# RIKEN-RCCS/EigenExa

Hardware: AMD Instinct MI355X
Metric: eigen_sx full-solve throughput (reference flop model: 4/3 N^3 + D&C GEMM + 2 nvec N^2) (higher is better)
Workload: dtype f64; 1 GPU; N=8192 random symmetric fp64 (counter-based R+R^T, seed 20240807), eigen_sx all eigenpairs, m_forward=64, m_backward=128; parallelism=1 GPU (1x1 grid)

## Files before the change

### eigenexa_amd/csrc/api.hip

```cpp
#include "eigx_context.h"
#include "eigx_comm.h"
#include "../../include/eigenexa_amd.h"
#include <cstring>

namespace eigx {
Context g_ctx;
}

using namespace eigx;

extern "C" {

int eigx_init(int device) {
  return eigx_init_multi(device, 0, 1, nullptr, 'C');
}

int eigx_get_device_count(void) {
  int ndev = 0;
  if (hipGetDeviceCount(&ndev) != hipSuccess) { (void)hipGetLastError(); return 0; }
  return ndev;
}

int eigx_get_rccl_unique_id(void* out128) {
  return comm_get_unique_id(out128);
// ... 269 lines not shown
  for (size_t q = 0; q < g_ctx.prof_kind.size(); ++q) {
    const int k = g_ctx.prof_kind[q];
    if (k < 0 || k >= nkinds) continue;
    float ms = 0.f;
    EIGX_HIP_CHECK(hipEventElapsedTime(&ms, g_ctx.prof_ev[2 * q], g_ctx.prof_ev[2 * q + 1]));
    out[3 * k + 0] += 1.0;
    out[3 * k + 1] += g_ctx.prof_units[q];
    out[3 * k + 2] += 1e-3 * ms;
  }
  return EIGX_OK;
}

int eigx_device_synchronize(void) {
  if (!g_ctx.initialized) return EIGX_ERR_NOT_INITIALIZED;
  EIGX_HIP_CHECK(hipSetDevice(g_ctx.device));
  EIGX_HIP_CHECK(hipDeviceSynchronize());
  return EIGX_OK;
}

void* eigx_malloc_dev(int64_t bytes) {
  if (!g_ctx.initialized) return nullptr;
  void* p = nullptr;
  if (hipMalloc(&p, (size_t)bytes) != hipSuccess) return nullptr;
  return p;
}
int eigx_free_dev(void* p) {
  if (p) EIGX_HIP_CHECK(hipFree(p));
  return EIGX_OK;
}
int eigx_memcpy_h2d(void* dst, const void* src, int64_t bytes) {
  EIGX_HIP_CHECK(hipMemcpy(dst, src, (size_t)bytes, hipMemcpyHostToDevice));
  return EIGX_OK;
}
int eigx_memcpy_d2h(void* dst, const void* src, int64_t bytes) {
  EIGX_HIP_CHECK(hipMemcpy(dst, src, (size_t)bytes, hipMemcpyDeviceToHost));
  return EIGX_OK;
}

int eigx_tune(int key, int value) {
  if (key == 0) return set_gemm_variant(value);
  if (key == 1) return set_bisect_threads(value);
  if (key == 2) return set_bt_q(value);
  if (key == 3 || key == 4 || key == 5 || key == 10 || key == 11) return set_reduce_knob(key, value);
  if (key == 6) return set_gemm_cstream(value);
  if (key == 7) return value > 0 ? set_reduce_knob(key, value) : -1;
  if (key == 8) return set_dc_chunk(value);
  if (key == 9) return comm_set_bounce(value);
  if (key == 15) return set_dc_pipe(value);
  if (key == 16) return set_dc_batch(value);
  if (key == 17 || key == 18 || key == 19) return set_range_knob(key, value);
  if (key == 20) return set_tri_nb(value);
  if (key == 21) return set_batch_nmax(value);
  if (key == 22) return set_hbatch_nmax(value);
  return -1;
}

int eigx_dgemm_dev(char opa, char opb, int m, int n, int k, double alpha, const double* a, int lda,
                   const double* b, int ldb, double beta, double* c, int ldc, int tri_upper) {
  if (!g_ctx.initialized) return EIGX_ERR_NOT_INITIALIZED;
  EIGX_HIP_CHECK(hipStreamSynchronize(nullptr));
  dgemm_dev(g_ctx.stream, opa, opb, m, n, k, alpha, a, lda, b, ldb, beta, c, ldc, tri_upper ? 1 : 0,
            &g_ctx.grid);
  EIGX_HIP_CHECK(hipStreamSynchronize(g_ctx.stream));
  return EIGX_OK;
}

int eigx_dgemm_gather_dev(char opa, char opb, int m, int n, int k, double alpha, const double* a, int lda,
                          const double* b, int ldb, double beta, double* c, int ldc, const int* kmap_a,
                          const int* kmap_b) {
  if (!g_ctx.initialized) return EIGX_ERR_NOT_INITIALIZED;
  EIGX_HIP_CHECK(hipStreamSynchronize(nullptr));
  dgemm_dev(g_ctx.stream, opa, opb, m, n, k, alpha, a, lda, b, ldb, beta, c, ldc, 0, nullptr, kmap_a, nullptr, 1, 0,
            0, 0, 1, 0, 0, 0, 1, 0, kmap_b);
  EIGX_HIP_CHECK(hipStreamSynchronize(g_ctx.stream));
  return EIGX_OK;
}

}
```

### eigenexa_amd/csrc/dc.hip

```cpp
#include "eigx_context.h"
#include "eigx_comm.h"
#include "../../include/eigenexa_amd.h"
#include <algorithm>
#include <cfloat>
#include <cstring>

namespace eigx {

namespace {

constexpr int LEAF = 32;

constexpr int LEAF_T = 64;
__global__ __launch_bounds__(LEAF_T) void jacobi_leaf_kernel(const double* __restrict__ d,
                                                             const double* __restrict__ e, int lde, int band,
                                                             const int* __restrict__ leaf_off,
                                                             const int* __restrict__ leaf_n, double* __restrict__ D,
                                                             double* __restrict__ Q, int ldq, int r0, int r1) {
  __shared__ double A[LEAF][LEAF + 1];
  __shared__ double V[LEAF][LEAF + 1];
  __shared__ double cs[LEAF / 2][2];
  __shared__ int pq[LEAF / 2][2];
  __shared__ int perm[LEAF];
  const int tid = threadIdx.x;
// ... 202 lines not shown
  const int jj = blockIdx.x * blockDim.x + threadIdx.x;
  if (jj >= M.nm) return;
  double v = 0.0;
  if (jj < M.K) {
    const int nch = (M.K + ZN_IC - 1) / ZN_IC;
    for (int c = 0; c < nch; ++c) v += zp[(size_t)c * ldn + M.off + jj];
  } else {
    const double* col = Qa + (size_t)dsrc[M.off + jj] * ldq;
    for (int t = 0; t < M.zr_n; ++t) v += M.zr_w[t] * col[M.zr_row[t]];
  }
  z[M.off + jj] = v;
}

__global__ void pack_rows_kernel(const double* __restrict__ Q, int ldq, int n, int r0, int nr, int rp,
                                 double* __restrict__ out) {
  const int j = blockIdx.y;
  for (int r = blockIdx.x * blockDim.x + threadIdx.x; r < rp; r += gridDim.x * blockDim.x)
    out[(size_t)j * rp + r] = (r < nr) ? Q[(size_t)j * ldq + r0 + r] : 0.0;
}
__global__ void unpack_rows_kernel(const double* __restrict__ in, int n, int rp, double* __restrict__ Q, int ldq) {
  const int j = blockIdx.y, q = blockIdx.z;
  const double* src = in + (size_t)q * rp * n + (size_t)j * rp;
  for (int r = blockIdx.x * blockDim.x + threadIdx.x; r < rp; r += gridDim.x * blockDim.x)
    if (q * rp + r < n) Q[(size_t)j * ldq + q * rp + r] = src[r];
}

template <int CTRL>
__device__ __forceinline__ double dc_dpp_add(double v) {
  const int lo2 = __builtin_amdgcn_update_dpp(0, __double2loint(v), CTRL, 0xf, 0xf, true);
  const int hi2 = __builtin_amdgcn_update_dpp(0, __double2hiint(v), CTRL, 0xf, 0xf, true);
  return v + __hiloint2double(hi2, lo2);
}

__device__ __forceinline__ double dc_swapadd16(double v) {
  const auto lo = __builtin_amdgcn_permlane16_swap(__double2loint(v), __double2loint(v), false, false);
  const auto hi = __builtin_amdgcn_permlane16_swap(__double2hiint(v), __double2hiint(v), false, false);
  return __hiloint2double(hi[0], lo[0]) + __hiloint2double(hi[1], lo[1]);
}

__device__ __forceinline__ double group8_sum(double v) {
  v = dc_dpp_add<0xB1>(v);
  v = dc_dpp_add<0x4E>(v);
  v = dc_dpp_add<0x141>(v);
  return v;
}

template <int LPR>
__device__ __forceinline__ double group_sum(double v) {
  v = group8_sum(v);
  if (LPR == 32) { v = dc_dpp_add<0x140>(v); v = dc_swapadd16(v); }
  return v;
}

template <int LPR>
__global__ __launch_bounds__(256) void secular_kernel(const MergeDev* __restrict__ md,
                                                      const double* __restrict__ dlam,
                                                      const double* __restrict__ wz, double* __restrict__ Dn,
                                                      double* __restrict__ S, int lds, int P, int rank,
                                                      double* __restrict__ sec, int nsec) {
  const MergeDev M = md[blockIdx.y];
  const int K = M.K;
  constexpr int RPW = 256 / LPR;
  __shared__ double so[RPW], stau[RPW];
  const int jbase = (P > 1) ? (int)((long)K * rank / P) : 0;
  const int jend = (P > 1) ? (int)((long)K * (rank + 1) / P) : K;
  if (jbase + (int)(blockIdx.x * RPW) >= jend) return;
  const int sub = threadIdx.x & (LPR - 1);
  const int jraw = jbase + blockIdx.x * RPW + threadIdx.x / LPR;
  const bool act = jraw < jend;
  const int j = act ? jraw : K - 1;
  const double* __restrict__ d = dlam + M.off;
  const double* __restrict__ z = wz + M.off;
  double* Sp = S + (size_t)M.off * lds + M.off;
  const double rho = M.rho, rhoinv = 1.0 / rho;
  const double eps = DBL_EPSILON / 2.0;
  if (K == 1) {
    if (threadIdx.x == 0) {
      const double t = rho * z[0] * z[0];
      if (sec) { sec[M.off] = d[0] + t; sec[nsec + M.off] = d[0]; sec[2 * nsec + M.off] = t; }
      else { Dn[M.off] = d[0] + t; Sp[0] = -t; }
    }
    return;
  }
  const bool last = (j == K - 1);
  const int jl = last ? K - 2 : j, jr = jl + 1;
  double origin, lo, hi, tau;
  {
    const double gap = last ? rho : d[j + 1] - d[j];
    const double base = last ? d[K - 1] : d[j], half = 0.5 * gap;
    double c = 0.0;
    for (int i = sub; i < K; i += LPR)
      if (i != jl && i != jr) c += z[i] * z[i] / ((d[i] - base) - half);
    c = group_sum<LPR>(c) + rhoinv;
    const double zl2 = z[jl] * z[jl], zr2 = z[jr] * z[jr];
    const double fmid = c + zl2 / ((d[jl] - base) - half) + zr2 / ((d[jr] - base) - half);
    int org;
    if (last) { org = K - 1; if (fmid <= 0.0) { lo = 0.5 * gap; hi = gap; } else { lo = 0.0; hi = 0.5 * gap; } }
    else if (fmid > 0.0) { org = j; lo = 0.0; hi = 0.5 * gap; }
    else { org = j + 1; lo = -0.5 * gap; hi = 0.0; }
    origin = d[org];
    const double dl = d[jl] - origin, dr = d[jr] - origin;
    const double qa = c, qb = -(c * (dl + dr) + zl2 + zr2), qc = c * dl * dr + zl2 * dr + zr2 * dl;
    tau = 0.5 * (lo + hi);
    const double disc = qb * qb - 4.0 * qa * qc;
    if (disc >= 0.0) {
      const double sq = sqrt(disc);
      const double qq = -0.5 * (qb + (qb >= 0.0 ? sq : -sq));
      const double r1 = (qa != 0.0) ? qq / qa : NAN, r2 = (qq != 0.0) ? qc / qq : NAN;
      if (r1 > lo && r1 < hi) tau = r1;
      else if (r2 > lo && r2 < hi) tau = r2;
    }
  }
  for (int iter = 0; iter < 100; ++iter) {
    double psi = 0.0, dpsi = 0.0, phi = 0.0, dphi = 0.0, err = 0.0;
    for (int i = sub; i < K; i += LPR) {
      const double t = z[i] / ((d[i] - origin) - tau);
      const double zt = z[i] * t, tt = t * t;
      if (i <= jl) { psi += zt; dpsi += tt; err += fabs(psi); }
      else { phi += zt; dphi += tt; err += fabs(phi); }
    }
    psi = group_sum<LPR>(psi); dpsi = group_sum<LPR>(dpsi);
    phi = group_sum<LPR>(phi); dphi = group_sum<LPR>(dphi);
    err = group_sum<LPR>(err);
    const double wv = rhoinv + phi + psi;
    err = 8.0 * (fabs(phi) + fabs(psi)) + err + 2.0 * rhoinv + fabs(tau) * (dpsi + dphi);
    if (fabs(wv) <= eps * err) break;
    if (wv < 0.0) lo = tau; else hi = tau;
    const double Dl = (d[jl] - origin) - tau, Dr = (d[jr] - origin) - tau;
    const double aa = (Dl + Dr) * wv - Dl * Dr * (dpsi + dphi);
    const double bb = Dl * Dr * wv;
    const double cc = wv - Dl * dpsi - Dr * dphi;
    double eta;
    {
      double disc = aa * aa - 4.0 * bb * cc;
      if (disc < 0.0) disc = 0.0;
      const double sq = sqrt(disc);
      if (cc == 0.0) eta = (aa != 0.0) ? bb / aa : 0.0;
      else if (aa <= 0.0) eta = (aa - sq) / (2.0 * cc);
      else eta = 2.0 * bb / (aa + sq);
    }
    if (wv * eta >= 0.0) eta = -wv / (dpsi + dphi);
    double tnew = tau + eta;
    if (!(tnew > lo && tnew < hi)) tnew = 0.5 * (lo + hi);
    if (tnew == tau) break;
    tau = tnew;
  }
  if (sec) {
    if (sub == 0 && act) { sec[M.off + j] = origin + tau; sec[nsec + M.off + j] = origin; sec[2 * nsec + M.off + j] = tau; }
    return;
  }
  if (sub == 0) { so[threadIdx.x / LPR] = origin; stau[threadIdx.x / LPR] = tau; if (act) Dn[M.off + j] = origin + tau; }
  __syncthreads();
  {
    const int r = threadIdx.x % RPW, ii = threadIdx.x / RPW;
    const int jr = blockIdx.x * RPW + r;
    if (jr < K) {
      const double o_ = so[r], t_ = stau[r];
      for (int i = ii; i < K; i += 256 / RPW) Sp[jr + (size_t)i * lds] = (d[i] - o_) - t_;
    }
  }
}

__global__ __launch_bounds__(256) void loewner_kernel(const MergeDev* __restrict__ md,
                                                      const double* __restrict__ dlam,
                                                      const double* __restrict__ wz, const double* __restrict__ S,
                                                      int lds, double* __restrict__ zh) {
  const MergeDev M = md[blockIdx.y];
  const int K = M.K;
  const int lane = threadIdx.x & 63;
  const int i = blockIdx.x * 4 + (threadIdx.x >> 6);
  if (i >= K) return;
  const double* d = dlam + M.off;
  const double* Sp = S + (size_t)M.off * lds + M.off + (size_t)i * lds;
  const double di = d[i];
  double prod = 1.0;
  for (int j = lane; j < K; j += 64) {
    const double num = -Sp[j];
    prod *= (j == i) ? num : num / (d[j] - di);
  }
  for (int o = 32; o > 0; o >>= 1) prod *= __shfl_xor(prod, o, 64);
  if (lane == 0) {
    const double v = sqrt(fabs(prod));
    zh[M.off + i] = (wz[M.off + i] >= 0.0) ? v : -v;
  }
}

constexpr int VEC_IC = 256;
__global__ __launch_bounds__(256) void vectors1_kernel(const MergeDev* __restrict__ md, const double* __restrict__ zh,
                                                       double* __restrict__ S, int lds, double* __restrict__ vnp,
                                                       int ldn) {
  __shared__ double part[4][64];
  const MergeDev M = md[blockIdx.z];
  const int K = M.K;
  if ((int)(blockIdx.x * 64) >= K || (int)(blockIdx.y * VEC_IC) >= K) return;
  const int lane = threadIdx.x & 63, wave = threadIdx.x >> 6;
  const int j = blockIdx.x * 64 + lane;
  const bool act = j < K;
  double* Sp = S + (size_t)M.off * lds + M.off + j;
  const double* zz = zh + M.off;
  const int i0 = blockIdx.y * VEC_IC;
  const int i1 = (i0 + VEC_IC < K) ? i0 + VEC_IC : K;
  double nrm = 0.0;
  if (act)
    for (int i = i0 + wave; i < i1; i += 4) {
      const double v = zz[i] / Sp[(size_t)i * lds];
      Sp[(size_t)i * lds] = v;
      nrm += v * v;
    }
  part[wave][lane] = nrm;
  __syncthreads();
  if (wave == 0 && act)
    vnp[(size_t)blockIdx.y * ldn + M.off + j] = (part[0][lane] + part[1][lane]) + (part[2][lane] + part[3][lane]);
}
__global__ __launch_bounds__(256) void vectors2_kernel(const MergeDev* __restrict__ md, double* __restrict__ S, int lds,
                                                       const double* __restrict__ vnp, int ldn) {
  const MergeDev M = md[blockIdx.z];
  const int K = M.K;
  if ((int)(blockIdx.x * 64) >= K || (int)(blockIdx.y * VEC_IC) >= K) return;
  const int lane = threadIdx.x & 63, wave = threadIdx.x >> 6;
  const int j = blockIdx.x * 64 + lane;
  if (j >= K) return;
  const int nch = (K + VEC_IC - 1) / VEC_IC;
  double nrm = 0.0;
  for (int c = 0; c < nch; ++c) nrm += vnp[(size_t)c * ldn + M.off + j];
  const double sc = 1.0 / sqrt(nrm);
  double* Sp = S + (size_t)M.off * lds + M.off + j;
  const int i0 = blockIdx.y * VEC_IC;
  const int i1 = (i0 + VEC_IC < K) ? i0 + VEC_IC : K;
  for (int i = i0 + wave; i < i1; i += 4) Sp[(size_t)i * lds] *= sc;
}

__global__ void scatter_lambda_kernel(const MergeDev* __restrict__ md, const double* __restrict__ sec, double* __restrict__ Dn) {
  const MergeDev M = md[blockIdx.y];
  const int j = blockIdx.x * blockDim.x + threadIdx.x;
  if (j < M.K) Dn[M.off + j] = sec[M.off + j];
}
__global__ __launch_bounds__(256) void loewner_mg_kernel(const MergeDev* __restrict__ md, const double* __restrict__ dlam,
                                                         const double* __restrict__ wz, const double* __restrict__ sec,
                                                         int nsec, double* __restrict__ zh) {
  const MergeDev M = md[blockIdx.y];
  const int K = M.K;
  const int lane = threadIdx.x & 63;
  const int i = blockIdx.x * 4 + (threadIdx.x >> 6);
  if (i >= K) return;
  const double* d = dlam + M.off;
  const double* org = sec + nsec + M.off;
  const double* tau = sec + 2 * nsec + M.off;
  const double di = d[i];
  double prod = 1.0;
  for (int j = lane; j < K; j += 64) {
    const double num = (org[j] - di) + tau[j];
    prod *= (j == i) ? num : num / (d[j] - di);
  }
  for (int o = 32; o > 0; o >>= 1) prod *= __shfl_xor(prod, o, 64);
  if (lane == 0) {
    const double v = sqrt(fabs(prod));
    zh[M.off + i] = (wz[M.off + i] >= 0.0) ? v : -v;
  }
}
__global__ __launch_bounds__(256) void vectors_mg_kernel(const MergeDev* __restrict__ md, int mi0, const double* __restrict__ dlam,
                                                         const double* __restrict__ zh, const double* __restrict__ sec, int nsec,
                                                         int j0, int j1, int compact, double* __restrict__ Sc, int ldsc) {
  __shared__ double part[4][64];
  const MergeDev M = md[mi0 + blockIdx.z];
  const int K = M.K;
  const int jhi = (j1 < K) ? j1 : K;
  const int lane = threadIdx.x & 63, wave = threadIdx.x >> 6;
  const int j = j0 + blockIdx.x * 64 + lane;
  if (j0 + (int)(blockIdx.x * 64) >= jhi) return;
  const bool act = j < jhi;
  const double* d = dlam + M.off;
  const double* zz = zh + M.off;
  const double oj = act ? sec[nsec + M.off + j] : 0.0, tj = act ? sec[2 * nsec + M.off + j] : 1.0;
  double nrm = 0.0;
  for (int i = wave; i < K; i += 4) {
    const double v = zz[i] / ((d[i] - oj) - tj);
    nrm += v * v;
  }
  part[wave][lane] = nrm;
  __syncthreads();
  const double sc = 1.0 / sqrt((part[0][lane] + part[1][lane]) + (part[2][lane] + part[3][lane]));
  if (!act) return;
// ... 99 lines not shown
        }
      nodes[id].sig[k] = sig[k];
      for (int r = 0; r < band; ++r) {
        nodes[id].wv[k][r] = y[band * k + r];
        nodes[id].wv[k][band + r] = x[band * k + r];
      }
    }
    const int l = build(off, n1);
    const int r = build(off + n1, nn - n1);
    nodes[id].left = l; nodes[id].right = r;
    nodes[l].parent = id; nodes[r].parent = id;
    nodes[id].height = 1 + std::max(nodes[l].height, nodes[r].height);
    return id;
  }
};

void sort_index_runs(const double* d, int nm, std::vector<int>& idx, std::vector<int>& tmp, std::vector<int>& bounds) {
  idx.resize(nm);
  for (int i = 0; i < nm; ++i) idx[i] = i;
  bounds.clear();
  bounds.push_back(0);
  for (int i = 1; i < nm; ++i)
    if (d[i] < d[i - 1]) bounds.push_back(i);
  bounds.push_back(nm);
  auto cmp = [d](int a, int b) { return d[a] < d[b] || (d[a] == d[b] && a < b); };
  int nr = (int)bounds.size() - 1;
  if (nr > 16) { std::sort(idx.begin(), idx.end(), cmp); return; }
  tmp.resize(nm);
  while (nr > 1) {
    int w = 0;
    for (int r = 0; r < nr; r += 2) {
      if (r + 1 < nr)
        std::merge(idx.begin() + bounds[r], idx.begin() + bounds[r + 1], idx.begin() + bounds[r + 1], idx.begin() + bounds[r + 2],
                   tmp.begin() + bounds[r], cmp);
      else
        std::copy(idx.begin() + bounds[r], idx.begin() + bounds[r + 1], tmp.begin() + bounds[r]);
      bounds[w++] = bounds[r];
    }
    bounds[w] = nm;
    nr = w;
    idx.swap(tmp);
  }
}

}

int g_dc_pipe = 1, g_dc_batch = 1, g_dc_side_min = 1024;
int set_dc_pipe(int v) {
  const int old = g_dc_pipe;
  if (v >= 2) g_dc_side_min = v; else g_dc_pipe = v ? 1 : 0;
  return old;
}
int set_dc_batch(int v) { const int old = g_dc_batch; g_dc_batch = v ? 1 : 0; return old; }
int g_dc_chunk = 2048;
int set_dc_chunk(int v) {
  const int old = g_dc_chunk;
  if (v >= 64 && v <= 2048 && v % 64 == 0) g_dc_chunk = v;
  return old;
}

void band_dc_prepare(Context& ctx, int n) {
  const int P = ctx.grid.nranks;
  const int ldq = (P > 1) ? pad_ld((n + P - 1) / P + 2) : pad_ld(n);
  double* Qa = ctx.pool.get_t<double>("dc.Qa", (size_t)ldq * n);
  double* Qb = ctx.pool.get_t<double>("dc.Qb", (size_t)ldq * n);
  EIGX_HIP_CHECK(hipMemsetAsync(Qa, 0, (size_t)ldq * n * 8, ctx.side_stream));
  EIGX_HIP_CHECK(hipMemsetAsync(Qb, 0, (size_t)ldq * n * 8, ctx.side_stream));
  EIGX_HIP_CHECK(hipEventRecord(ctx.dc_ev, ctx.side_stream));
  ctx.dc_zero_n = n; ctx.dc_zero_qa = Qa; ctx.dc_zero_qb = Qb;
}

void band_dc_dev(Context& ctx, int n, int nvec, const double* d_dev, const double* e_dev, int lde, int band,
                 double* w_dev, double* z_dev, int ldz, const std::function<void()>& side_work) {
  hipStream_t st = ctx.stream;
  const double eps = DBL_EPSILON / 2.0;
  const int P = ctx.grid.nranks;
  const int rp = (n + P - 1) / P;
  const int r0 = P > 1 ? std::min(n, ctx.grid.rank * rp) : 0;
  const int r1 = P > 1 ? std::min(n, r0 + rp) : n;
  auto clip = [&](int lo, int hi, int& a, int& b) { a = std::max(lo, r0); b = std::min(hi, r1); return b > a; };
  HostDC H;
  H.n = n; H.band = band; H.lde = lde;
  H.d.resize(n);
  H.e.resize((size_t)lde * band);
  EIGX_HIP_CHECK(hipMemcpyAsync(H.d.data(), d_dev, (size_t)n * 8, hipMemcpyDeviceToHost, st));
  EIGX_HIP_CHECK(hipMemcpyAsync(H.e.data(), e_dev, (size_t)lde * band * 8, hipMemcpyDeviceToHost, st));
  EIGX_HIP_CHECK(hipStreamSynchronize(st));
  double nrm = 0.0;
  for (int i = 0; i < n; ++i) {
    nrm = std::max(nrm, fabs(H.d[i]));
    for (int b = 1; b <= band; ++b) if (i >= b) nrm = std::max(nrm, fabs(H.E(i, b)));
  }
  const double scl = nrm > 0.0 ? 1.0 / nrm : 1.0;
  for (int i = 0; i < n; ++i) {
    H.d[i] *= scl;
    for (int b = 1; b <= band; ++b) H.E(i, b) = (i >= b) ? H.E(i, b) * scl : 0.0;
  }
  H.nodes.reserve(2 * (n / (LEAF / 2) + 2));
  const int root = H.build(0, n);
  const int maxh = H.nodes[root].height;

  const bool pipe = (P == 1) && g_dc_pipe;
  const int ldq = (P > 1) ? pad_ld(rp + 2) : pad_ld(n);
  double* Qa_base = ctx.pool.get_t<double>("dc.Qa", (size_t)ldq * n);
  double* Qb_base = ctx.pool.get_t<double>("dc.Qb", (size_t)ldq * n);
  double* Qa = Qa_base - r0;
  double* Qb = Qb_base - r0;
  const int SCW = g_dc_chunk;
  const int lds_mg = SCW;
  double* Sbuf[2];
  Sbuf[0] = ctx.pool.get_t<double>("dc.S", (P > 1) ? (size_t)n * SCW + 64 : (size_t)ldq * n);
  Sbuf[1] = pipe ? ctx.pool.get_t<double>("dc.S2", (size_t)ldq * n) : Sbuf[0];
  double* sec = (P > 1) ? ctx.pool.get_t<double>("dc.sec", (size_t)3 * n) : nullptr;
  double* dd = ctx.pool.get_t<double>("dc.d", (size_t)n);
  double* de = ctx.pool.get_t<double>("dc.e", (size_t)lde * band);
  double* zh = ctx.pool.get_t<double>("dc.zh", (size_t)n);
  double* vnp = ctx.pool.get_t<double>("dc.vnp", (size_t)n * ((n + VEC_IC - 1) / VEC_IC + 1));
  double* zp = pipe ? ctx.pool.get_t<double>("dc.zp", (size_t)n * ((n + ZN_IC - 1) / ZN_IC + 1)) : nullptr;
  const int maxmerge = n / (LEAF / 2) + 8;
  int* leafinfo = ctx.pool.get_t<int>("dc.leaf", (size_t)2 * maxmerge);
  int* perm_dev = ctx.pool.get_t<int>("dc.perm", (size_t)n);
  int* iota_dev = ctx.pool.get_t<int>("dc.iota", (size_t)n);
  struct Arena {
    char *dev, *host;
    MergeDev *md_dev, *md_h;
    GemmBatch *gb_dev, *gb_h;
    int *nd_dev, *nd_h, *rpj_dev, *rpj_h, *rjj_dev, *rjj_h, *cps_dev, *cps_h, *cpd_dev, *cpd_h, *cpr_dev, *cpr_h, *cpn_dev, *cpn_h;
    int *topA_dev, *topA_h, *topB_dev, *topB_h, *botA_dev, *botA_h, *botB_dev, *botB_h, *dsrc_dev, *dsrc_h;
    double *dlam, *dl_h, *wz, *wz_h, *rc_dev, *rc_h, *rs_dev, *rs_h, *Dcur, *Dh, *zbuf, *zhost;
  } ar[2];
  const size_t npad = ((size_t)n + 7) / 8 * 8;
  const size_t md_bytes = ((size_t)maxmerge * sizeof(MergeDev) + 63) / 64 * 64;
  const size_t gb_bytes = ((size_t)2 * maxmerge * sizeof(GemmBatch) + 63) / 64 * 64;
  const size_t up_bytes = md_bytes + gb_bytes + 12 * npad * sizeof(int) + 5 * npad * sizeof(double);
  const size_t arena_bytes = up_bytes + npad * sizeof(double);
  const size_t down_off = up_bytes - npad * 8;
  {
    char* dev_all = (char*)ctx.pool.get("dc.arena", 2 * arena_bytes);
    char* host_all = (char*)ctx.pool.get_host("dc.arena", 2 * arena_bytes);
    memset(host_all, 0, 2 * arena_bytes);
    for (int q = 0; q < 2; ++q) {
      Arena& A = ar[q];
      A.dev = dev_all + q * arena_bytes;
      A.host = host_all + q * arena_bytes;
      size_t pos = 0;
      auto carve = [&](size_t bytes, void* pd, void* ph) {
        *(char**)pd = A.dev + pos; *(char**)ph = A.host + pos; pos += bytes;
      };
      carve(md_bytes, &A.md_dev, &A.md_h);
      carve(gb_bytes, &A.gb_dev, &A.gb_h);
      carve(npad * 4, &A.nd_dev, &A.nd_h);
      carve(npad * 4, &A.rpj_dev, &A.rpj_h);  carve(npad * 4, &A.rjj_dev, &A.rjj_h);
      carve(npad * 4, &A.cps_dev, &A.cps_h);  carve(npad * 4, &A.cpd_dev, &A.cpd_h);
      carve(npad * 4, &A.cpr_dev, &A.cpr_h);  carve(npad * 4, &A.cpn_dev, &A.cpn_h);
      carve(npad * 4, &A.topA_dev, &A.topA_h); carve(npad * 4, &A.topB_dev, &A.topB_h);
      carve(npad * 4, &A.botA_dev, &A.botA_h); carve(npad * 4, &A.botB_dev, &A.botB_h);
      carve(npad * 4, &A.dsrc_dev, &A.dsrc_h);
      carve(npad * 8, &A.dlam, &A.dl_h);  carve(npad * 8, &A.wz, &A.wz_h);
      carve(npad * 8, &A.rc_dev, &A.rc_h); carve(npad * 8, &A.rs_dev, &A.rs_h);
      carve(npad * 8, &A.Dcur, &A.Dh);    carve(npad * 8, &A.zbuf, &A.zhost);
    }
  }
  MergeDev* md_h2 = (MergeDev*)ctx.pool.get_host("dc.md2", md_bytes);

  EIGX_HIP_CHECK(hipMemcpyAsync(dd, H.d.data(), (size_t)n * 8, hipMemcpyHostToDevice, st));
  EIGX_HIP_CHECK(hipMemcpyAsync(de, H.e.data(), (size_t)lde * band * 8, hipMemcpyHostToDevice, st));
// ... 207 lines not shown
      const unsigned nmg = (unsigned)ids.size();
      hipStream_t sb = (pipe && maxnm > g_dc_side_min) ? ctx.dc_stream : st;
      const bool batched = (P == 1) && g_dc_batch && maxK > 0 && mds.size() > 1 &&
                           (long)ceil_div(maxnm, 128) * ceil_div(maxK, 128) < 192;
      int nbatch = 0, bmaxM = 0;
      if (batched) {
        const int bot_shift = (int)(C.botA_dev - C.topA_dev);
        for (size_t q = 0; q < mds.size(); ++q) {
          const MergeDev& M = mds[q];
          if (M.K <= 0) continue;
          auto add = [&](int row0, int rows, int kk, int offKA, int offKB) {
            if (rows <= 0) return;
            GemmBatch& B = C.gb_h[nbatch++];
            B.M = rows; B.N = M.K; B.K = kk; B.pad = 0;
            B.offA = row0; B.offB = (long)M.off * ldq + M.off; B.offC = (long)M.off * ldq + row0;
            B.offKA = offKA; B.offKB = offKB;
            bmaxM = std::max(bmaxM, rows);
          };
          if (k == 0) {
            add(M.off, M.n1, ktop[q], M.off, M.off);
            add(M.off + M.n1, M.nm - M.n1, kbot[q], M.off + bot_shift, M.off + bot_shift);
            gemm_flops += 2.0 * (double)M.K * ((double)M.n1 * ktop[q] + (double)(M.nm - M.n1) * kbot[q]);
          } else {
            add(M.off, M.nm, M.K, M.off, 0);
            gemm_flops += 2.0 * M.nm * (double)M.K * M.K;
          }
        }
      }
      const double tt2 = trace ? now_s() : 0.0;
      double t_gemm_enq = 0.0;
      memcpy(C.md_h, mds.data(), mds.size() * sizeof(MergeDev));
      EIGX_HIP_CHECK(hipMemcpyAsync(C.dev, C.host, up_bytes, hipMemcpyHostToDevice, sb));
      const bool mg = P > 1;
      const bool compact = mg && maxnm <= lds_mg;
      if (maxK > 0) {
        if (mg) {
          const int kmx = maxK / P + 2;
          EIGX_HIP_CHECK(hipMemsetAsync(sec, 0, (size_t)3 * n * 8, st));
          if (maxK >= 512)
            hipLaunchKernelGGL(secular_kernel<32>, dim3((kmx + 7) / 8, nmg), dim3(256), 0, st, C.md_dev, C.dlam, C.wz, C.Dcur, S, ldq, P,
                               ctx.grid.rank, sec, n);
          else
            hipLaunchKernelGGL(secular_kernel<8>, dim3((kmx + 31) / 32, nmg), dim3(256), 0, st, C.md_dev, C.dlam, C.wz, C.Dcur, S, ldq, P,
                               ctx.grid.rank, sec, n);
          comm_allreduce_sum(ctx, COMM_WORLD, sec, (size_t)3 * n, st);
          hipLaunchKernelGGL(scatter_lambda_kernel, dim3((maxK + 255) / 256, nmg), dim3(256), 0, st, C.md_dev, sec, C.Dcur);
          hipLaunchKernelGGL(loewner_mg_kernel, dim3((maxK + 3) / 4, nmg), dim3(256), 0, st, C.md_dev, C.dlam, C.wz, sec, n, zh);
          if (compact)
            hipLaunchKernelGGL(vectors_mg_kernel, dim3((maxK + 63) / 64, 1, nmg), dim3(256), 0, st, C.md_dev, 0, C.dlam, zh, sec, n, 0,
                               maxK, 1, S, lds_mg);
        } else {
          if (maxK >= 512)
            hipLaunchKernelGGL(secular_kernel<32>, dim3((maxK + 7) / 8, nmg), dim3(256), 0, sb, C.md_dev, C.dlam, C.wz, C.Dcur, S, ldq, 1, 0,
                               (double*)nullptr, 0);
          else
            hipLaunchKernelGGL(secular_kernel<8>, dim3((maxK + 31) / 32, nmg), dim3(256), 0, sb, C.md_dev, C.dlam, C.wz, C.Dcur, S, ldq, 1, 0,
                               (double*)nullptr, 0);
          hipLaunchKernelGGL(loewner_kernel, dim3((maxK + 3) / 4, nmg), dim3(256), 0, sb, C.md_dev, C.dlam, C.wz, S, ldq, zh);
          const dim3 vg((maxK + 63) / 64, (maxK + VEC_IC - 1) / VEC_IC, nmg);
          hipLaunchKernelGGL(vectors1_kernel, vg, dim3(256), 0, sb, C.md_dev, zh, S, ldq, vnp, n);
          hipLaunchKernelGGL(vectors2_kernel, vg, dim3(256), 0, sb, C.md_dev, S, ldq, vnp, n);
        }
      }
      if (sb != st) {
        EIGX_HIP_CHECK(hipEventRecord(ctx.dc_b_ev, sb));
        EIGX_HIP_CHECK(hipStreamWaitEvent(st, ctx.dc_b_ev, 0));
      }
      if (pipe && pi + 1 == passes.size()) {
        EIGX_HIP_CHECK(hipMemcpyAsync(V.Dh, C.Dcur, (size_t)n * 8, hipMemcpyDeviceToHost, sb));
        EIGX_HIP_CHECK(hipEventRecord(ctx.dc_z_ev, sb));
        early_final = V.Dh;
      }
      if (nrot > 0)
        hipLaunchKernelGGL(rotate_kernel, dim3((maxnm + 255) / 256, nmg), dim3(256), 0, st, C.md_dev,
                           C.rpj_dev, C.rjj_dev, C.rc_dev, C.rs_dev, Qa, ldq, r0, r1);
      if (z_ahead) {
        if (maxK > 0)
          hipLaunchKernelGGL(znext1_kernel, dim3((maxK + 63) / 64, (maxK + ZN_IC - 1) / ZN_IC, nmg), dim3(256), 0, st, C.md_dev,
                             C.nd_dev, Qa, ldq, S, ldq, zp, n);
        hipLaunchKernelGGL(znext2_kernel, dim3((maxnm + 255) / 256, nmg), dim3(256), 0, st, C.md_dev, C.dsrc_dev, Qa, ldq, zp, n,
                           C.zbuf);
        EIGX_HIP_CHECK(hipMemcpyAsync(C.host + down_off, C.dev + down_off, 2 * npad * 8, hipMemcpyDeviceToHost, st));
        EIGX_HIP_CHECK(hipEventRecord(ctx.dc_z_ev, st));
        z_ready = true;
      }
      if (pi + 1 == passes.size()) run_side_work();
      if (maxK > 0) {
        const bool fan = mds.size() > 1 && !(mg && !compact) && !batched;
        if (fan) {
          EIGX_HIP_CHECK(hipEventRecord(ctx.aux_ev[Context::kAux], st));
          for (int q = 0; q < Context::kAux; ++q) EIGX_HIP_CHECK(hipStreamWaitEvent(ctx.aux[q], ctx.aux_ev[Context::kAux], 0));
        }
        int rr = 0;
        const double tg0 = trace ? now_s() : 0.0;
        if (batched) {
          if (k == 0)
            dgemm_gather_batch_dev(st, C.gb_dev, nbatch, bmaxM, maxK, Qa, ldq, S, ldq, Qb, ldq, C.topA_dev, C.topB_dev);
          else
            dgemm_gather_batch_dev(st, C.gb_dev, nbatch, bmaxM, maxK, Qa, ldq, S, ldq, Qb, ldq, C.nd_dev, iota_dev);
        } else
        for (size_t q = 0; q < mds.size(); ++q) {
          const MergeDev& M = mds[q];
          if (M.K <= 0) continue;
          const bool chunked = mg && !compact;
          int cwq = M.K;
          if (chunked) { cwq = (int)(((size_t)n * SCW / (size_t)M.K) / 64 * 64); if (cwq > M.K) cwq = M.K; if (cwq < 64) cwq = 64; }
          for (int j0 = 0; j0 < M.K; j0 += cwq) {
          const int cw = (M.K - j0 < cwq) ? M.K - j0 : cwq;
          const int ldsb = mg ? (chunked ? ((cw + 1) & ~1) : lds_mg) : ldq;
          const double* Sb = mg ? (chunked ? S : S + (size_t)M.off * lds_mg) : S + (size_t)M.off * ldq + M.off;
          if (chunked) {
            hipLaunchKernelGGL(vectors_mg_kernel, dim3((cw + 63) / 64, 1, 1), dim3(256), 0, st, C.md_dev, (int)q, C.dlam, zh, sec, n, j0,
                               j0 + cw, 0, S, ldsb);
          }
// ... 113 lines not shown
```

### eigenexa_amd/csrc/eigx_common.h

```cpp
#pragma once
#include <hip/hip_runtime.h>
#include <cstdio>
#include <cstdlib>
#include <cstdint>
#include <cmath>
#include <vector>
#include <ctime>
#include <chrono>

#define EIGX_HIP_CHECK(expr)                                                        \
  do {                                                                              \
    hipError_t _e = (expr);                                                         \
    if (_e != hipSuccess) {                                                         \
      fprintf(stderr, "[eigx] HIP error %s at %s:%d: %s\n", hipGetErrorName(_e),    \
              __FILE__, __LINE__, hipGetErrorString(_e));                           \
      abort();                                                                      \
    }                                                                               \
  } while (0)

namespace eigx {

typedef double d4_t __attribute__((ext_vector_type(4)));

struct Grid {
// ... 38 lines not shown
struct SolveRequest {
  char mode;
  int nvec;
  bool want_vec;
};
inline char upper_case(char c) { return (c >= 'a' && c <= 'z') ? (char)(c - 'a' + 'A') : c; }
inline SolveRequest normalize_request(int n, int nvec, char mode) {
  mode = upper_case(mode);
  if (nvec == 0) mode = 'N';
  if (nvec < 0) nvec = -nvec;
  if (nvec > n) nvec = n;
  return SolveRequest{mode, nvec, mode != 'N'};
}


__global__ void fill_kernel(double* p, size_t n, double v);
__global__ void fill_vec_kernel(double* __restrict__ w, int n, double v);
__global__ void scale_vec_kernel(double* __restrict__ w, int n, double s);

void dgemm_dev(hipStream_t stream, char opA, char opB, int M, int N, int K, double alpha,
               const double* A, int lda, const double* B, int ldb, double beta, double* C, int ldc,
               int tri_mode = 0, const Grid* g = nullptr, const int* kmapA = nullptr,
               const int* cmapC = nullptr, int batch = 1, long strideA = 0, long strideB = 0, long strideC = 0,
               int batch2 = 1, long strideA2 = 0, long strideB2 = 0, long strideC2 = 0, int ownP = 1,
               int ownp = 0, const int* kmapB = nullptr, int tn_lo = 0, int tn_hi = 0x7fffffff);

struct GemmBatch {
  int M, N, K, pad;
  long offA, offB, offC;
  int offKA, offKB;
};
void dgemm_gather_batch_dev(hipStream_t stream, const GemmBatch* tab_dev, int nbatch, int maxM, int maxN,
                            const double* A, int lda, const double* B, int ldb, double* C, int ldc,
                            const int* kmapA, const int* kmapB);

inline void stage_trace(int rank, const char* what, long detail = -1) {
  static const bool on = getenv("EIGX_TRACE_STAGES") != nullptr;
  if (!on) return;
  timespec ts;
  clock_gettime(CLOCK_MONOTONIC, &ts);
  if (detail >= 0) fprintf(stderr, "[eigx stage] rank %d t=%.3f %s %ld\n", rank, ts.tv_sec % 100000 + ts.tv_nsec * 1e-9, what, detail);
  else fprintf(stderr, "[eigx stage] rank %d t=%.3f %s\n", rank, ts.tv_sec % 100000 + ts.tv_nsec * 1e-9, what);
  fflush(stderr);
}

int set_gemm_variant(int v);
int set_gemm_cstream(int v);
int set_bisect_threads(int v);
int set_bt_q(int v);
int set_reduce_knob(int key, int v);
int set_dc_chunk(int v);
int set_dc_pipe(int v);
int set_dc_batch(int v);
int set_batch_nmax(int v);
int set_hbatch_nmax(int v);

}
```

Baseline: 18840 GFLOP/s.

## Stage secular poles in LDS and recompute D&C vectors from secular triples

The secular solver now streams the d and z poles through double-buffered shared-memory chunks, unrolled by four. All rows in a block keep iterating until a block-wide live flag clears. On a single GPU the secular kernel now writes (lambda, origin, tau) triples, and the Loewner and vector kernels recompute each eigenvector entry from those triples instead of reading and writing the S matrix that secular_kernel used to fill. The aim is to cut global-memory traffic in the D&C merge. The cost is extra __syncthreads and redundant iterations for rows that have already converged.

```diff
diff --git a/eigenexa_amd/csrc/api.hip b/eigenexa_amd/csrc/api.hip
--- a/eigenexa_amd/csrc/api.hip
+++ b/eigenexa_amd/csrc/api.hip
@@ -345,6 +345,7 @@
   if (key == 20) return set_tri_nb(value);
   if (key == 21) return set_batch_nmax(value);
   if (key == 22) return set_hbatch_nmax(value);
+  if (key == 23) return set_dc_triples(value);
   return -1;
 }
 
diff --git a/eigenexa_amd/csrc/dc.hip b/eigenexa_amd/csrc/dc.hip
--- a/eigenexa_amd/csrc/dc.hip
+++ b/eigenexa_amd/csrc/dc.hip
@@ -278,6 +278,62 @@
   return v;
 }
 
+constexpr int SEC_CH = 512;
+constexpr int SEC_U = 4;
+
+#define SEC_KEEP(a) _Pragma("unroll") for (int u_ = 0; u_ < SEC_U; ++u_) asm volatile("" : "+v"(a[u_]))
+
+template <int LPR>
+__device__ __forceinline__ void secular_mid_chunk(const double* __restrict__ cd, const double* __restrict__ cz, int c0, int K,
+                                                  int sub, int jl, int jr, double base, double half, double& c) {
+#pragma clang fp contract(off)
+  static_assert(SEC_CH % (SEC_U * LPR) == 0, "a lane's groups of SEC_U poles tile the stage");
+  for (int m = sub; m < SEC_CH; m += SEC_U * LPR) {
+    if (c0 + m >= K) break;
+    double q[SEC_U];
+#pragma unroll
+    for (int u = 0; u < SEC_U; ++u) {
+      const double dv = cd[m + u * LPR], zv = cz[m + u * LPR];
+      q[u] = zv * zv / ((dv - base) - half);
+    }
+    SEC_KEEP(q);
+#pragma unroll
+    for (int u = 0; u < SEC_U; ++u) {
+      const int i = c0 + m + u * LPR;
+      if (i < K && i != jl && i != jr) c += q[u];
+    }
+  }
+}
+
+template <int LPR>
+__device__ __forceinline__ void secular_eval_chunk(const double* __restrict__ cd, const double* __restrict__ cz, int c0, int K,
+                                                   int sub, int jl, double origin, double tau, double& psi, double& dpsi,
+                                                   double& phi, double& dphi, double& err) {
+#pragma clang fp contract(off)
+  for (int m = sub; m < SEC_CH; m += SEC_U * LPR) {
+    if (c0 + m >= K) break;
+    double zv[SEC_U], t[SEC_U];
+#pragma unroll
+    for (int u = 0; u < SEC_U; ++u) {
+      const double dv = cd[m + u * LPR];
+      zv[u] = cz[m + u * LPR];
+      t[u] = zv[u] / ((dv - origin) - tau);
+    }
+    SEC_KEEP(t);
+#pragma unroll
+    for (int u = 0; u < SEC_U; ++u) {
+      const int i = c0 + m + u * LPR;
+      if (i < K) {
+        const double zt = zv[u] * t[u], tt = t[u] * t[u];
+        if (i <= jl) { psi += zt; dpsi += tt; err += fabs(psi); }
+        else { phi += zt; dphi += tt; err += fabs(phi); }
+      }
+    }
+  }
+}
+
+#undef SEC_KEEP
+
 template <int LPR>
 __global__ __launch_bounds__(256) void secular_kernel(const MergeDev* __restrict__ md,
                                                       const double* __restrict__ dlam,
@@ -288,6 +344,8 @@
   const int K = M.K;
   constexpr int RPW = 256 / LPR;
   __shared__ double so[RPW], stau[RPW];
+  __shared__ double sd[2][SEC_CH], sz[2][SEC_CH];
+  __shared__ int live[3];
   const int jbase = (P > 1) ? (int)((long)K * rank / P) : 0;
   const int jend = (P > 1) ? (int)((long)K * (rank + 1) / P) : K;
   if (jbase + (int)(blockIdx.x * RPW) >= jend) return;
@@ -304,10 +362,38 @@
     if (threadIdx.x == 0) {
       const double t = rho * z[0] * z[0];
       if (sec) { sec[M.off] = d[0] + t; sec[nsec + M.off] = d[0]; sec[2 * nsec + M.off] = t; }
-      else { Dn[M.off] = d[0] + t; Sp[0] = -t; }
+      else Sp[0] = -t;
+      if (P == 1) Dn[M.off] = d[0] + t;
     }
     return;
   }
+  constexpr int SPT = SEC_CH / 256;
+  const int nch = (K + SEC_CH - 1) / SEC_CH;
+  double pd[SPT], pz[SPT];
+  int cur = 0;
+  auto fetch = [&](int ch) {
+#pragma unroll
+    for (int s = 0; s < SPT; ++s) {
+      const int i = ch * SEC_CH + s * 256 + (int)threadIdx.x;
+      pd[s] = (i < K) ? d[i] : 0.0;
+      pz[s] = (i < K) ? z[i] : 0.0;
+    }
+  };
+  auto put = [&](int b) {
+#pragma unroll
+    for (int s = 0; s < SPT; ++s) { sd[b][s * 256 + threadIdx.x] = pd[s]; sz[b][s * 256 + threadIdx.x] = pz[s]; }
+  };
+  auto sweep = [&](auto&& body) {
+    for (int ch = 0; ch < nch; ++ch) {
+      if (nch > 1) fetch(ch + 1 < nch ? ch + 1 : 0);
+      body(sd[cur], sz[cur], ch * SEC_CH);
+      if (nch > 1) { put(cur ^ 1); __syncthreads(); cur ^= 1; }
+    }
+  };
+  fetch(0);
+  put(0);
+  if (threadIdx.x < 3) live[threadIdx.x] = 0;
+  __syncthreads();
   const bool last = (j == K - 1);
   const int jl = last ? K - 2 : j, jr = jl + 1;
   double origin, lo, hi, tau;
@@ -315,8 +401,7 @@
     const double gap = last ? rho : d[j + 1] - d[j];
     const double base = last ? d[K - 1] : d[j], half = 0.5 * gap;
     double c = 0.0;
-    for (int i = sub; i < K; i += LPR)
-      if (i != jl && i != jr) c += z[i] * z[i] / ((d[i] - base) - half);
+    sweep([&](const double* cd, const double* cz, int c0) { secular_mid_chunk<LPR>(cd, cz, c0, K, sub, jl, jr, base, half, c); });
     c = group_sum<LPR>(c) + rhoinv;
     const double zl2 = z[jl] * z[jl], zr2 = z[jr] * z[jr];
     const double fmid = c + zl2 / ((d[jl] - base) - half) + zr2 / ((d[jr] - base) - half);
@@ -337,42 +422,50 @@
       else if (r2 > lo && r2 < hi) tau = r2;
     }
   }
+  bool done = false;
   for (int iter = 0; iter < 100; ++iter) {
     double psi = 0.0, dpsi = 0.0, phi = 0.0, dphi = 0.0, err = 0.0;
-    for (int i = sub; i < K; i += LPR) {
-      const double t = z[i] / ((d[i] - origin) - tau);
-      const double zt = z[i] * t, tt = t * t;
-      if (i <= jl) { psi += zt; dpsi += tt; err += fabs(psi); }
-      else { phi += zt; dphi += tt; err += fabs(phi); }
-    }
-    psi = group_sum<LPR>(psi); dpsi = group_sum<LPR>(dpsi);
-    phi = group_sum<LPR>(phi); dphi = group_sum<LPR>(dphi);
-    err = group_sum<LPR>(err);
-    const double wv = rhoinv + phi + psi;
-    err = 8.0 * (fabs(phi) + fabs(psi)) + err + 2.0 * rhoinv + fabs(tau) * (dpsi + dphi);
-    if (fabs(wv) <= eps * err) break;
-    if (wv < 0.0) lo = tau; else hi = tau;
-    const double Dl = (d[jl] - origin) - tau, Dr = (d[jr] - origin) - tau;
-    const double aa = (Dl + Dr) * wv - Dl * Dr * (dpsi + dphi);
-    const double bb = Dl * Dr * wv;
-    const double cc = wv - Dl * dpsi - Dr * dphi;
-    double eta;
-    {
-      double disc = aa * aa - 4.0 * bb * cc;
-      if (disc < 0.0) disc = 0.0;
-      const double sq = sqrt(disc);
-      if (cc == 0.0) eta = (aa != 0.0) ? bb / aa : 0.0;
-      else if (aa <= 0.0) eta = (aa - sq) / (2.0 * cc);
-      else eta = 2.0 * bb / (aa + sq);
-    }
-    if (wv * eta >= 0.0) eta = -wv / (dpsi + dphi);
-    double tnew = tau + eta;
-    if (!(tnew > lo && tnew < hi)) tnew = 0.5 * (lo + hi);
-    if (tnew == tau) break;
-    tau = tnew;
+    sweep([&](const double* cd, const double* cz, int c0) {
+      if (!done) secular_eval_chunk<LPR>(cd, cz, c0, K, sub, jl, origin, tau, psi, dpsi, phi, dphi, err);
+    });
+    if (!done) {
+      psi = group_sum<LPR>(psi); dpsi = group_sum<LPR>(dpsi);
+      phi = group_sum<LPR>(phi); dphi = group_sum<LPR>(dphi);
+      err = group_sum<LPR>(err);
+      const double wv = rhoinv + phi + psi;
+      err = 8.0 * (fabs(phi) + fabs(psi)) + err + 2.0 * rhoinv + fabs(tau) * (dpsi + dphi);
+      if (fabs(wv) <= eps * err) done = true;
+      else {
+        if (wv < 0.0) lo = tau; else hi = tau;
+        const double Dl = (d[jl] - origin) - tau, Dr = (d[jr] - origin) - tau;
+        const double aa = (Dl + Dr) * wv - Dl * Dr * (dpsi + dphi);
+        const double bb = Dl * Dr * wv;
+        const double cc = wv - Dl * dpsi - Dr * dphi;
+        double eta;
+        {
+          double disc = aa * aa - 4.0 * bb * cc;
+          if (disc < 0.0) disc = 0.0;
+          const double sq = sqrt(disc);
+          if (cc == 0.0) eta = (aa != 0.0) ? bb / aa : 0.0;
+          else if (aa <= 0.0) eta = (aa - sq) / (2.0 * cc);
+          else eta = 2.0 * bb / (aa + sq);
+        }
+        if (wv * eta >= 0.0) eta = -wv / (dpsi + dphi);
+        double tnew = tau + eta;
+        if (!(tnew > lo && tnew < hi)) tnew = 0.5 * (lo + hi);
+        if (tnew == tau) done = true; else tau = tnew;
+      }
+    }
+    if (threadIdx.x == 0) live[(iter + 1) % 3] = 0;
+    if (!done) live[iter % 3] = 1;
+    __syncthreads();
+    if (!live[iter % 3]) break;
   }
   if (sec) {
-    if (sub == 0 && act) { sec[M.off + j] = origin + tau; sec[nsec + M.off + j] = origin; sec[2 * nsec + M.off + j] = tau; }
+    if (sub == 0 && act) {
+      sec[M.off + j] = origin + tau; sec[nsec + M.off + j] = origin; sec[2 * nsec + M.off + j] = tau;
+      if (P == 1) Dn[M.off + j] = origin + tau;
+    }
     return;
   }
   if (sub == 0) { so[threadIdx.x / LPR] = origin; stau[threadIdx.x / LPR] = tau; if (act) Dn[M.off + j] = origin + tau; }
@@ -431,7 +524,7 @@
     for (int i = i0 + wave; i < i1; i += 4) {
       const double v = zz[i] / Sp[(size_t)i * lds];
       Sp[(size_t)i * lds] = v;
-      nrm += v * v;
+      nrm = fma(v, v, nrm);
     }
   part[wave][lane] = nrm;
   __syncthreads();
@@ -454,6 +547,68 @@
   const int i0 = blockIdx.y * VEC_IC;
   const int i1 = (i0 + VEC_IC < K) ? i0 + VEC_IC : K;
   for (int i = i0 + wave; i < i1; i += 4) Sp[(size_t)i * lds] *= sc;
+}
+
+__global__ __launch_bounds__(256) void vectors_norm_kernel(const MergeDev* __restrict__ md, const double* __restrict__ dlam,
+                                                           const double* __restrict__ zh, const double* __restrict__ sec,
+                                                           int nsec, double* __restrict__ vnp, int ldn) {
+  __shared__ double ds[VEC_IC], zs[VEC_IC];
+  __shared__ double part[4][64];
+  const MergeDev M = md[blockIdx.z];
+  const int K = M.K;
+  if ((int)(blockIdx.x * 64) >= K || (int)(blockIdx.y * VEC_IC) >= K) return;
+  const int lane = threadIdx.x & 63, wave = threadIdx.x >> 6;
+  const int j = blockIdx.x * 64 + lane;
+  const bool act = j < K;
+  const int i0 = blockIdx.y * VEC_IC;
+  const int i1 = (i0 + VEC_IC < K) ? i0 + VEC_IC : K;
+  {
+    const int i = i0 + threadIdx.x;
+    ds[threadIdx.x] = (i < i1) ? dlam[M.off + i] : 0.0;
+    zs[threadIdx.x] = (i < i1) ? zh[M.off + i] : 0.0;
+  }
+  __syncthreads();
+  const double oj = act ? sec[nsec + M.off + j] : 0.0, tj = act ? sec[2 * nsec + M.off + j] : 1.0;
+  double nrm = 0.0;
+  if (act) {
+#pragma unroll 4
+    for (int i = i0 + wave; i < i1; i += 4) {
+      const double v = zs[i - i0] / ((ds[i - i0] - oj) - tj);
+      nrm = fma(v, v, nrm);
+    }
+  }
+  part[wave][lane] = nrm;
+  __syncthreads();
+  if (wave == 0 && act)
+    vnp[(size_t)blockIdx.y * ldn + M.off + j] = (part[0][lane] + part[1][lane]) + (part[2][lane] + part[3][lane]);
+}
+__global__ __launch_bounds__(256) void vectors_store_kernel(const MergeDev* __restrict__ md, const double* __restrict__ dlam,
+                                                            const double* __restrict__ zh, const double* __restrict__ sec,
+                                                            int nsec, const double* __restrict__ vnp, int ldn,
+                                                            double* __restrict__ S, int lds) {
+  __shared__ double ds[VEC_IC], zs[VEC_IC];
+  const MergeDev M = md[blockIdx.z];
+  const int K = M.K;
+  if ((int)(blockIdx.x * 64) >= K || (int)(blockIdx.y * VEC_IC) >= K) return;
+  const int lane = threadIdx.x & 63, wave = threadIdx.x >> 6;
+  const int j = blockIdx.x * 64 + lane;
+  const int i0 = blockIdx.y * VEC_IC;
+  const int i1 = (i0 + VEC_IC < K) ? i0 + VEC_IC : K;
+  {
+    const int i = i0 + threadIdx.x;
+    ds[threadIdx.x] = (i < i1) ? dlam[M.off + i] : 0.0;
+    zs[threadIdx.x] = (i < i1) ? zh[M.off + i] : 0.0;
+  }
+  __syncthreads();
+  if (j >= K) return;
+  const int nch = (K + VEC_IC - 1) / VEC_IC;
+  double nrm = 0.0;
+  for (int c = 0; c < nch; ++c) nrm += vnp[(size_t)c * ldn + M.off + j];
+  const double sc = 1.0 / sqrt(nrm);
+  const double oj = sec[nsec + M.off + j], tj = sec[2 * nsec + M.off + j];
+  double* Sp = S + (size_t)M.off * lds + M.off + j;
+#pragma unroll 4
+  for (int i = i0 + wave; i < i1; i += 4) Sp[(size_t)i * lds] = zs[i - i0] / ((ds[i - i0] - oj) - tj) * sc;
 }
 
 __global__ void scatter_lambda_kernel(const MergeDev* __restrict__ md, const double* __restrict__ sec, double* __restrict__ Dn) {
@@ -659,6 +814,8 @@
   return old;
 }
 int set_dc_batch(int v) { const int old = g_dc_batch; g_dc_batch = v ? 1 : 0; return old; }
+int g_dc_triples = 1;
+int set_dc_triples(int v) { const int old = g_dc_triples; g_dc_triples = v ? 1 : 0; return old; }
 int g_dc_chunk = 2048;
 int set_dc_chunk(int v) {
   const int old = g_dc_chunk;
@@ -718,7 +875,8 @@
   double* Sbuf[2];
   Sbuf[0] = ctx.pool.get_t<double>("dc.S", (P > 1) ? (size_t)n * SCW + 64 : (size_t)ldq * n);
   Sbuf[1] = pipe ? ctx.pool.get_t<double>("dc.S2", (size_t)ldq * n) : Sbuf[0];
-  double* sec = (P > 1) ? ctx.pool.get_t<double>("dc.sec", (size_t)3 * n) : nullptr;
+  const bool triples = (P > 1) || g_dc_triples;
+  double* sec = triples ? ctx.pool.get_t<double>("dc.sec", (size_t)3 * n) : nullptr;
   double* dd = ctx.pool.get_t<double>("dc.d", (size_t)n);
   double* de = ctx.pool.get_t<double>("dc.e", (size_t)lde * band);
   double* zh = ctx.pool.get_t<double>("dc.zh", (size_t)n);
@@ -1032,14 +1190,20 @@
         } else {
           if (maxK >= 512)
             hipLaunchKernelGGL(secular_kernel<32>, dim3((maxK + 7) / 8, nmg), dim3(256), 0, sb, C.md_dev, C.dlam, C.wz, C.Dcur, S, ldq, 1, 0,
-                               (double*)nullptr, 0);
+                               sec, n);
           else
             hipLaunchKernelGGL(secular_kernel<8>, dim3((maxK + 31) / 32, nmg), dim3(256), 0, sb, C.md_dev, C.dlam, C.wz, C.Dcur, S, ldq, 1, 0,
-                               (double*)nullptr, 0);
-          hipLaunchKernelGGL(loewner_kernel, dim3((maxK + 3) / 4, nmg), dim3(256), 0, sb, C.md_dev, C.dlam, C.wz, S, ldq, zh);
+                               sec, n);
           const dim3 vg((maxK + 63) / 64, (maxK + VEC_IC - 1) / VEC_IC, nmg);
-          hipLaunchKernelGGL(vectors1_kernel, vg, dim3(256), 0, sb, C.md_dev, zh, S, ldq, vnp, n);
-          hipLaunchKernelGGL(vectors2_kernel, vg, dim3(256), 0, sb, C.md_dev, S, ldq, vnp, n);
+          if (triples) {
+            hipLaunchKernelGGL(loewner_mg_kernel, dim3((maxK + 3) / 4, nmg), dim3(256), 0, sb, C.md_dev, C.dlam, C.wz, sec, n, zh);
+            hipLaunchKernelGGL(vectors_norm_kernel, vg, dim3(256), 0, sb, C.md_dev, C.dlam, zh, sec, n, vnp, n);
+            hipLaunchKernelGGL(vectors_store_kernel, vg, dim3(256), 0, sb, C.md_dev, C.dlam, zh, sec, n, vnp, n, S, ldq);
+          } else {
+            hipLaunchKernelGGL(loewner_kernel, dim3((maxK + 3) / 4, nmg), dim3(256), 0, sb, C.md_dev, C.dlam, C.wz, S, ldq, zh);
+            hipLaunchKernelGGL(vectors1_kernel, vg, dim3(256), 0, sb, C.md_dev, zh, S, ldq, vnp, n);
+            hipLaunchKernelGGL(vectors2_kernel, vg, dim3(256), 0, sb, C.md_dev, S, ldq, vnp, n);
+          }
         }
       }
       if (sb != st) {
diff --git a/eigenexa_amd/csrc/eigx_common.h b/eigenexa_amd/csrc/eigx_common.h
--- a/eigenexa_amd/csrc/eigx_common.h
+++ b/eigenexa_amd/csrc/eigx_common.h
@@ -114,6 +114,7 @@
 int set_dc_chunk(int v);
 int set_dc_pipe(int v);
 int set_dc_batch(int v);
+int set_dc_triples(int v);
 int set_batch_nmax(int v);
 int set_hbatch_nmax(int v);
 
```

New measurement: 18880 GFLOP/s, median of 6. Within noise of the previous version (+0.2%).
